# AILab-UniFI/GNN-TableExtraction

Measured on AMD Instinct MI355X. Metric: nodes/sec (fwd+bwd node classification) on PubLayNet page graphs, higher is better.
Workload: dtype f32 (GEMM operands split exactly into 3 bf16 pieces, fp32 accumulate)

## Files before the change

### gnn-tableextraction_amd/_lib.py

```python
from __future__ import annotations

import ctypes
import os
from ctypes import POINTER, c_char_p, c_float, c_int, c_int64, c_uint64, c_void_p

_HERE = os.path.dirname(os.path.abspath(__file__))
LIB_PATH = os.environ.get("GTE_LIB_PATH") or os.path.join(_HERE, "libgte_hip.so")

SIGNATURES = {
    "gte_version": (c_int, []),
    "gte_last_error": (c_char_p, []),
    "gte_device_info": (c_int, [c_void_p, c_void_p, c_void_p, c_void_p, c_int]),
    "gte_spmm_csr": (c_int, [c_void_p, c_void_p, c_void_p, c_void_p, c_int64, c_void_p, c_int64,
                             c_int64, c_int64, c_int, c_int, c_void_p]),
    "gte_spmm_csr_accumulate": (c_int, [c_void_p, c_void_p, c_void_p, c_void_p, c_int64, c_void_p, c_int64,
                                        c_int64, c_int64, c_int, c_int, c_void_p]),
    "gte_spmm_csr_edge_workspace_bytes": (c_int64, [c_int64, c_int64]),
    "gte_spmm_csr_edge": (c_int, [c_void_p, c_void_p, c_void_p, c_void_p, c_int64, c_void_p, c_int64, c_int64, c_int64, c_int64, c_int,
                                  c_void_p, c_int64, c_void_p]),
    "gte_spmm_tile_rows": (c_int, []),
    "gte_spmm_csr_tiled": (c_int, [c_void_p, c_void_p, c_void_p, c_void_p, c_void_p, c_void_p, c_void_p, c_int64,
                                   c_void_p, c_int64, c_int64, c_int64, c_int, c_int, c_void_p]),
    "gte_coo_to_csr_workspace_bytes": (c_int64, [c_int64, c_int64]),
    "gte_coo_to_csr": (c_int, [c_void_p, c_void_p, c_void_p, c_void_p, c_int64, c_int64,
# ... 68 lines not shown
                                        c_void_p, c_int64, c_int64, c_void_p]),
    "gte_sage_narrow_bwd_ln_p3_pad": (c_int, [c_void_p, c_int64, c_void_p, c_int64, c_void_p, c_int64, c_int64, c_int64, c_void_p, c_int64,
                                              c_int64, c_void_p, c_int64, c_void_p, c_int64, c_void_p, c_int64, c_void_p, c_int64, c_void_p,
                                              c_int64, c_void_p, c_float, c_void_p, c_void_p, c_int64, c_void_p, c_void_p, c_void_p, c_int,
                                              c_void_p, c_void_p, c_void_p, c_void_p, c_int64, c_void_p]),
    "gte_gemm_p3_nt_ln_bwd_supported": (c_int, [c_int64]),
    "gte_gemm_p3_nt_ln_bwd_workspace_bytes": (c_int64, [c_int64, c_int64]),
    "gte_gemm_p3_nt_ln_bwd": (c_int, [c_void_p, c_int64, c_int64, c_void_p, c_int64, c_int64, c_void_p, c_int64, c_void_p, c_int64,
                                      c_void_p, c_void_p, c_void_p, c_int, c_void_p, c_int64, c_void_p, c_int64, c_void_p, c_void_p,
                                      c_void_p, c_int64, c_int64, c_void_p, c_int64, c_void_p]),
    "gte_gemm_p3_nt_smallk_bwd_supported": (c_int, [c_int64, c_int64]),
    "gte_gemm_p3_nt_smallk_bwd_workspace_bytes": (c_int64, [c_int64, c_int64, c_int64]),
    "gte_gemm_p3_nt_smallk_bwd": (c_int, [c_void_p, c_int64, c_int64, c_void_p, c_int64, c_int64, c_void_p, c_int64, c_void_p, c_int64,
                                          c_int64, c_void_p, c_int64, c_int64, c_void_p, c_int64, c_void_p, c_void_p, c_void_p, c_void_p,
                                          c_int, c_void_p, c_int64, c_void_p, c_void_p, c_void_p, c_int64, c_int64, c_void_p, c_int64,
                                          c_void_p]),
    "gte_gemm_p3_nt_rows": (c_int, [c_void_p, c_int64, c_int64, c_void_p, c_int64, c_void_p, c_int64, c_void_p, c_int64,
                                    c_void_p, c_int64, c_int64, c_int64, c_int, c_int, c_void_p]),
    "gte_gemm_p3_tn_rows": (c_int, [c_void_p, c_int64, c_void_p, c_int64, c_void_p, c_int64, c_void_p, c_int64, c_int64, c_void_p,
                                    c_int64, c_int64, c_int64, c_int64, c_void_p, c_int64, c_void_p]),
    "gte_gemm_p3_nt_rows2": (c_int, [c_void_p, c_int64, c_void_p, c_int64, c_int64, c_void_p, c_int64, c_void_p, c_int64, c_void_p,
                                     c_int64, c_void_p, c_int64, c_int64, c_int64, c_int, c_int, c_void_p]),
    "gte_gemm_p3_tn_rows2": (c_int, [c_void_p, c_int64, c_void_p, c_int64, c_void_p, c_int64, c_void_p, c_int64, c_int64, c_void_p,
                                     c_int64, c_int64, c_int64, c_int64, c_void_p, c_int64, c_void_p]),
    "gte_gemm_p3_nt_ln_fwd_supported": (c_int, [c_int64]),
    "gte_gemm_p3_nt_ln_fwd": (c_int, [c_void_p, c_int64, c_int64, c_void_p, c_int64, c_int64, c_void_p, c_int64, c_void_p, c_void_p,
                                      c_void_p, c_float, c_int, c_void_p, c_int64, c_void_p, c_int64, c_void_p, c_int64, c_void_p,
                                      c_int64, c_int64, c_void_p]),
    "gte_gemm_p3_nt_rows2_ln_fwd": (c_int, [c_void_p, c_int64, c_void_p, c_int64, c_int64, c_void_p, c_int64, c_void_p, c_int64, c_void_p,
                                            c_void_p, c_void_p, c_float, c_int, c_void_p, c_int64, c_void_p, c_int64, c_void_p, c_int64,
                                            c_void_p, c_int64, c_int64, c_void_p]),
    "gte_gemm_p3_set_rows64": (c_int, [c_int]),
    "gte_gemm_p3_nt_plan": (c_int, [c_int64, c_int64, c_int64, c_int64, c_int, c_int, c_int, ctypes.POINTER(c_int)]),
    "gte_gemm_p3_set_nt_cfg": (c_int, [c_int]),
    "gte_gemm_p3_set_ln_rows": (c_int, [c_int]),
    "gte_batch_assemble_defer": (c_int, [c_int]),
    "gte_head_dlq_finish_workspace_bytes": (c_int64, [c_int64]),
    "gte_head_dlq_finish": (c_int, [c_void_p, c_void_p, c_void_p, c_void_p, c_int64, c_int64, c_int64, c_void_p, c_float, c_void_p,
                                    c_void_p, c_int64, c_void_p, c_void_p, c_int64, c_void_p]),
    "gte_gemm_p3_tn_workspace_bytes": (c_int64, [c_int64, c_int64, c_int64, c_int64]),
    "gte_gemm_p3_tn": (c_int, [c_void_p, c_int64, c_void_p, c_int64, c_void_p, c_int64, c_void_p, c_int64, c_int64, c_void_p,
                               c_int64, c_int64, c_int64, c_int64, c_void_p, c_int64, c_void_p]),
    "gte_adam_ticket_bytes": (c_int64, []),
    "gte_gcnsage_step": (c_int, [c_void_p, c_int, POINTER(c_int), c_void_p]),
    "gte_gcnsage_step_wide_layers": (c_int, [c_void_p]),
    "gte_gcnsage_forward": (c_int, [c_void_p, c_void_p]),
    "gte_fold_defer_begin": (c_int, [c_void_p]),
    "gte_fold_defer_flush": (c_int, []),
    "gte_fold_defer_flush_adam": (c_int, [c_void_p, c_void_p, c_void_p, c_void_p, c_int64, c_void_p, c_void_p, c_void_p, POINTER(c_int)]),
    "gte_fold_defer_flush_adam_images": (c_int, [c_void_p, c_void_p, c_void_p, c_void_p, c_int64, c_void_p, c_void_p, c_void_p, c_void_p,
                                                 c_int, POINTER(c_int)]),
    "gte_sage_transform_fwd": (c_int, [c_void_p, c_int64, c_int64, c_void_p, c_int64, c_void_p, c_int64, c_void_p, c_int64,
                                       c_int64, c_void_p]),
    "gte_sage_qform_dw_workspace_bytes": (c_int64, [c_int64, c_int64, c_int64]),
    "gte_sage_qform_dw": (c_int, [c_void_p, c_int64, c_void_p, c_int64, c_void_p, c_int64, c_int64, c_void_p, c_int64,
                                  c_int64, c_int64, c_void_p, c_int64, c_void_p]),
    "gte_sage_qform_dx": (c_int, [c_void_p, c_int64, c_void_p, c_int64, c_void_p, c_int64, c_int64, c_int64, c_void_p,
                                  c_int64, c_int64, c_void_p]),
    "gte_sage_narrow_supported": (c_int, [c_int64, c_int64]),
    "gte_sage_narrow_fwd": (c_int, [c_void_p, c_int64, c_int64, c_void_p, c_int64, c_void_p, c_int64, c_void_p, c_int64,
                                    c_void_p, c_int64, c_int64, c_void_p]),
    "gte_sage_narrow_fwd_ln_supported": (c_int, [c_int64, c_int64]),
    "gte_sage_narrow_fwd_ln": (c_int, [c_void_p, c_int64, c_int64, c_void_p, c_void_p, c_float, c_int, c_void_p, c_int64, c_void_p,
                                       c_void_p, c_int64, c_void_p, c_int64, c_void_p, c_int64, c_void_p, c_int64, c_int64,
                                       c_void_p]),
    "gte_sage_narrow_bwd_workspace_bytes": (c_int64, [c_int64, c_int64, c_int64]),
# ... 157 lines not shown
```

### gnn-tableextraction_amd/csrc/gemm_p3.hip

```cpp
#include "gte_common.h"
#include "gemm_p3_host.h"
#include "p3.h"
#include "smallk_step.h"

#include <stdlib.h>
#include <type_traits>
#include <utility>

namespace {

typedef __bf16 bf16x8 __attribute__((ext_vector_type(8)));
typedef float f32x16 __attribute__((ext_vector_type(16)));
typedef short s16x4 __attribute__((ext_vector_type(4)));
typedef __attribute__((address_space(3))) void* lds_ptr_t;
constexpr unsigned SRD_FLAGS = 0x00020000u;

template <typename F, int... I>
__device__ __forceinline__ void static_for_impl(F&& f, std::integer_sequence<int, I...>) {
    (f(std::integral_constant<int, I>{}), ...);
}
template <int N, typename F>
__device__ __forceinline__ void static_for(F&& f) {
    static_for_impl(static_cast<F&&>(f), std::make_integer_sequence<int, N>{});
}
// ... 532 lines not shown
                const long long rg = row_base + rlk;
                if (lane < kk && rlk < SR && rg < M) { p.lnf_stats[rg] = st_mean; p.lnf_stats[M + rg] = st_rstd; }
            }
        }
    } else {
        asm volatile("s_barrier" ::: "memory");
        static_assert(BN == 256, "whole rows per workgroup");
        constexpr int SR = TM * 32, LDT = 256;
        float* tile = reinterpret_cast<float*>(lds);
        constexpr bool MSK = LNB == 3;
        const int n = p.N, M = p.M;
        const int j4 = 4 * lane;
        const bool okc = MSK ? j4 < ((n + 3) & ~3) : j4 < n;
        bool oke[4];
        float gam[4], bet[4], s_dg[4], s_db[4], s_dbias[4];
#pragma unroll
        for (int e = 0; e < 4; ++e) {
            oke[e] = MSK ? j4 + e < n : okc;
            gam[e] = oke[e] ? p.ln_gamma[j4 + e] : 1.f;
            bet[e] = oke[e] ? p.ln_beta[j4 + e] : 0.f;
            s_dg[e] = s_db[e] = s_dbias[e] = 0.f;
        }
        const float inv_n = 1.0f / (float)n;
        const int col_l = lane & 31, hrow = (lane >> 5) * 4;
        constexpr int RF = 4;
        constexpr bool PRE = WM == 1;
        constexpr int RPW = PRE ? SR / NW : 1;
        constexpr int PD = RPW <= 12 ? RPW : 8;
        float zpre[PD][4], mpre[PD], rpre[PD];
        auto request_row = [&](int slot, int k) {
            const int rg = m0 + wave + k * NW;
            const int rc = rg < M ? rg : min(m0, M - 1);
            f4u zt; zt.x = zt.y = zt.z = zt.w = 0.f;
            if (okc) zt = *reinterpret_cast<const f4u*>(p.ln_z + (long long)rc * p.ln_ldz + j4);
            zpre[slot][0] = zt.x; zpre[slot][1] = zt.y; zpre[slot][2] = zt.z; zpre[slot][3] = zt.w;
            mpre[slot] = p.ln_stats[rc]; rpre[slot] = p.ln_stats[M + rc];
        };
        if constexpr (PRE) {
#pragma unroll
            for (int k = 0; k < PD; ++k) request_row(k, k);
        }
        for (int sl = 0; sl < WM; ++sl) {
            asm volatile("s_barrier" ::: "memory");
            if (wm == sl) {
#pragma unroll
                for (int b = 0; b < TN; ++b)
#pragma unroll
                    for (int a = 0; a < TM; ++a)
#pragma unroll
                        for (int r = 0; r < 16; ++r)
                            tile[(a * 32 + hrow + (r & 3) + 8 * (r >> 2)) * LDT + wn * (TN * 32) + b * 32 + col_l] = acc[a][b][r];
            }
            asm volatile("s_waitcnt lgkmcnt(0)\n\ts_barrier" ::: "memory");
            const int row_base = m0 + sl * SR;
            constexpr int ROUNDS = (SR + RF * NW - 1) / (RF * NW);
#pragma unroll
            for (int rd = 0; rd < ROUNDS; ++rd) {
                const int rl = wave + rd * RF * NW;
                if (rl >= SR) break;
                float gy[RF][4], zz[RF][4], mean[RF], rstd[RF];
                bool rok[RF];
#pragma unroll
                for (int u = 0; u < RF; ++u) {
                    const int rloc = rl + u * NW, rg = row_base + rloc;
                    rok[u] = rloc < SR && rg < M;
                    const int rc = rok[u] ? rg : min(row_base, M - 1);
                    float4 a = make_float4(0.f, 0.f, 0.f, 0.f), bz = a;
                    if (okc) {
                        if (rok[u]) a = *reinterpret_cast<const float4*>(tile + rloc * LDT + j4);
// ... 4 lines not shown
                    }
                    gy[u][0] = a.x; gy[u][1] = a.y; gy[u][2] = a.z; gy[u][3] = a.w;
                    if constexpr (PRE) {
                        const int k = rd * RF + u;
                        const int e_ = (k < RPW ? k : 0) % PD;
#pragma unroll
                        for (int e = 0; e < 4; ++e) zz[u][e] = zpre[e_][e];
                        mean[u] = mpre[e_]; rstd[u] = rpre[e_];
                        if (k + PD < RPW) request_row(e_, k + PD);
                    } else {
                        zz[u][0] = bz.x; zz[u][1] = bz.y; zz[u][2] = bz.z; zz[u][3] = bz.w;
                        mean[u] = p.ln_stats[rc]; rstd[u] = p.ln_stats[M + rc];
                    }
                }
                float dd[RF][4];
#pragma unroll
                for (int u = 0; u < RF; ++u) {
#pragma unroll
                    for (int e = 0; e < 4; ++e) dd[u][e] = 0.f;
                    if (!rok[u]) continue;
                    const long long rg = row_base + rl + u * NW;
                    float xh[4], g[4];
                    float a = 0.f, b = 0.f;
                    if constexpr (MSK) gte_ln_bwd_pre4m(gy[u], zz[u], mean[u], rstd[u], gam, bet, oke, p.ln_relu, xh, g, a, b);
                    else gte_ln_bwd_pre4(gy[u], zz[u], mean[u], rstd[u], gam, bet, okc, p.ln_relu, xh, g, a, b);
                    const float c1 = gte_group_sum<64>(a) * inv_n, c2 = gte_group_sum<64>(b) * inv_n;
                    if constexpr (MSK) gte_ln_bwd_post4m(g, xh, gam, rstd[u], c1, c2, oke, dd[u], s_dg, s_db, s_dbias);
                    else gte_ln_bwd_post4(g, xh, gam, rstd[u], c1, c2, okc, dd[u], s_dg, s_db, s_dbias);
                    if (okc && p.ln_dz) {
                        f4u o; o.x = dd[u][0]; o.y = dd[u][1]; o.z = dd[u][2]; o.w = dd[u][3];
                        *reinterpret_cast<f4u*>(p.ln_dz + rg * p.ln_lddz + j4) = o;
                    }
                }
                if (p.ln_dzp3) {
                    const bool odd = lane & 1;
                    const int col0 = 4 * (lane & ~1);
                    const bool im8 = MSK ? col0 < ((n + 15) & ~15) : col0 < n;
#pragma unroll
                    for (int u = 0; u < RF; u += 2) {
                        float x[8];
#pragma unroll
                        for (int e = 0; e < 4; ++e) {
                            const float got = gte_quad_swap1(odd ? dd[u][e] : dd[u + 1][e]);
                            x[e] = odd ? got : dd[u][e];
                            x[4 + e] = odd ? dd[u + 1][e] : got;
                        }
                        if (im8 && rok[odd ? u + 1 : u])
                            p3::store8(p.ln_dzp3 + (long long)(row_base + rl + (odd ? u + 1 : u) * NW) * p.ln_ldp3, col0, x);
                    }
                }
            }
        }
        asm volatile("s_waitcnt lgkmcnt(0)\n\ts_barrier" ::: "memory");
        float* red = reinterpret_cast<float*>(lds);
#pragma unroll
        for (int e = 0; e < 4; ++e) {
            red[(wave * 3 + 0) * 256 + j4 + e] = s_dg[e];
            red[(wave * 3 + 1) * 256 + j4 + e] = s_db[e];
            red[(wave * 3 + 2) * 256 + j4 + e] = s_dbias[e];
        }
        asm volatile("s_waitcnt lgkmcnt(0)\n\ts_barrier" ::: "memory");
        float* pp = p.ln_part + (long long)lb * 3 * n;
        for (int i = tid; i < 3 * 256; i += NW * 64) {
            const int q = i >> 8, j = i & 255;
            float v = 0.f;
#pragma unroll
            for (int w = 0; w < NW; ++w) v += red[(w * 3 + q) * 256 + j];
            if (j < n) pp[q * n + j] = v;
        }
    }
}

template <int WM, int WN, int TM, int TN, int NL, int LNB = 0, bool BIG = false>
__global__ void __launch_bounds__((WM * WN + NL) * 64, (WM * WN + NL + 3) / 4)
gemm_p3_nt_lw_kernel(const P3Gemm p) {
    constexpr int NW = WM * WN, NBUF = 3;
    constexpr int BM = WM * TM * 32, BN = WN * TN * 32;
    constexpr int A_INST = BM * 96 / 1024, B_INST = BN * 96 / 1024, N_INST = A_INST + B_INST;
    constexpr int A_BYTES = BM * 96;
    constexpr int NI = (N_INST + NL - 1) / NL;
    constexpr int STAGE = NI * NL * 1024;
    extern __shared__ __attribute__((aligned(16))) char lds[];

// ... 121 lines not shown
#if P3_ABL & 16
    const long long c0 = __builtin_amdgcn_s_memtime(), r0 = __builtin_amdgcn_s_memrealtime();
#endif
#if P3_ABL & 4
    F f;
    read_frags(f, lds);
#endif
    for (int t = 0; t < T; ++t) {
#if !(P3_ABL & 4)
        F f;
        read_frags(f, lds + rd * STAGE);
#endif
#if P3_ABL & 8
        keep_frags<TM, TN>(f);
#else
        products<TM, TN>(acc, f);
#endif
        asm volatile("s_waitcnt lgkmcnt(0)\n\ts_barrier" ::: "memory");
        rd = rd + 1 == NBUF ? 0 : rd + 1;
    }
#if P3_ABL & 16
    if (tid == 0 && p.slab) {
        long long* st = reinterpret_cast<long long*>(p.slab) + 2 * blockIdx.x;
        st[0] = __builtin_amdgcn_s_memtime() - c0;
        st[1] = __builtin_amdgcn_s_memrealtime() - r0;
    }
#endif
#if P3_ABL & 32
    if (p.K != 12345) return;
#endif
    lw_epilogue<WM, WN, TM, TN, LNB>(acc, lds, p, m0, n0, lb, wave, lane, tid);
}

template <int TM, int NL, int LNB = 0, int SQ = 4>
__global__ void __launch_bounds__((8 + NL) * 64, (8 + NL + 3) / 4)
gemm_p3_nt_sq_kernel(const P3Gemm p) {
    constexpr int WM = 1, WN = 8, TN = 1, NW = 8, NSLOT = 3;
    constexpr int BM = TM * 32, BN = 256;
    constexpr int G = BM * 96 / 1024;
    constexpr int NG = (G + NL - 1) / NL;
    constexpr int NIQ = NG * SQ;
    constexpr int BLK = BM * 96, SLOT = SQ * BLK;
    static_assert(SQ == 4 && BLK % 1024 == 0 && NIQ <= 24, "slot");
    extern __shared__ __attribute__((aligned(16))) char lds[];

    const int tid = threadIdx.x, lane = tid & 63;
    const int wave = __builtin_amdgcn_readfirstlane(tid >> 6);
    const int tiles_n = (p.N + BN - 1) / BN;
    const unsigned lb = gte_xcd_remap(blockIdx.x, gridDim.x);
    const int tm = (int)(lb / (unsigned)tiles_n), tn = (int)(lb % (unsigned)tiles_n);
    const int m0 = tm * BM, n0 = tn * BN;
    const int KB1 = p.KB1, T = p.KB1 + p.KB2;
    const int S = (T + SQ - 1) / SQ;

    if (wave >= NW) {
        const int lw = wave - NW;
        const int rowsA = min(BM, p.M - m0);
        const int lda1 = (int)p.lda1, lda2 = (int)(p.A2 ? p.lda2 : p.lda1);
        const char* baseA1 = p.rowsA ? p.A1 : p.A1 + (long long)m0 * p.lda1;
        const char* baseA2 = p.A2 ? (p.rows_both ? p.A2 : p.A2 + (long long)m0 * p.lda2) : baseA1;
        const int recA1 = p.rowsA ? (int)(unsigned)p.res_bytes : rowsA * lda1;
        const int recA2 = p.rows_both ? (int)(unsigned)p.res_bytes2 : rowsA * lda2;
        constexpr int OOB = (int)0xfffffc00u;
        char* const scratch = lds + NSLOT * SLOT;
        int vo1[NG], vo2[NG];
        static_for<NG>([&](auto GI) {
            constexpr int g = decltype(GI)::value;
            const int gi = g * NL + lw;
            const int sl = gi * 64 + lane, row = sl / 6, part = sl - row * 6, sp = part ^ ((row >> 3) & 1);
            vo1[g] = gi >= G ? OOB : row * lda1 + sp * 16;
            vo2[g] = gi >= G ? OOB : row * lda2 + sp * 16;
            if (p.rowsA && gi < G) {
                const int rr = row < rowsA ? p.rowsA[m0 + row] : -1;
                vo1[g] = rr < 0 ? OOB : (int)((unsigned)rr * (unsigned)lda1 + (unsigned)(sp * 16));
                if (p.rows_both) vo2[g] = rr < 0 ? OOB : (int)((unsigned)rr * (unsigned)lda2 + (unsigned)(sp * 16));
            }
        });
        const __amdgpu_buffer_rsrc_t sa1 = __builtin_amdgcn_make_buffer_rsrc(const_cast<char*>(baseA1), 0, recA1, SRD_FLAGS);
        const __amdgpu_buffer_rsrc_t sa2 = __builtin_amdgcn_make_buffer_rsrc(const_cast<char*>(baseA2), 0, recA2, SRD_FLAGS);
        auto issue = [&](int s, char* slot) {
            static_for<NG>([&](auto GI) {
                constexpr int g = decltype(GI)::value;
                const int gi = g * NL + lw;
                static_for<SQ>([&](auto QI) {
                    constexpr int q = decltype(QI)::value;
#if P3_ABL & 1
                    if (s >= 2) return;
#endif
                    const int t = s * SQ + q;
                    const bool seg = t >= KB1;
                    const int vo = seg ? vo2[g] : vo1[g];
                    dma16(seg ? sa2 : sa1, gi < G ? slot + q * BLK + gi * 1024 : scratch,
                          (t < T && vo != OOB) ? vo + (seg ? t - KB1 : t) * 96 : OOB);
                });
            });
        };
        issue(0, lds);
        issue(1, lds + SLOT);
        wait_dma_barrier<NIQ>();
        int wr = 2;
        for (int s = 0; s < S; ++s) {
            issue(s + 2, lds + wr * SLOT);
            wr = wr + 1 == NSLOT ? 0 : wr + 1;
            wait_dma_barrier<NIQ>();
        }
        if constexpr (LNB != 0) asm volatile("s_waitcnt vmcnt(0)\n\ts_barrier" ::: "memory");
        return;
    }
    const int wn = wave;
    const int r = lane & 31, hsel = lane >> 5;
    const int a_rd = r * 96 + (hsel ^ ((r >> 3) & 1)) * 16;
    const int rowsB = min(BN, p.N - n0);
    const char* const baseB = p.B + (long long)n0 * 96;
    const int b_vo = (wn * 32 + r) * 96 + hsel * 16;
    const long long bsb = p.bsb;
    bf16x8 bq[4][3];
    auto load_b = [&](bf16x8 (&dst)[3], int t, bool valid) {
        const __amdgpu_buffer_rsrc_t sb = __builtin_amdgcn_make_buffer_rsrc(const_cast<char*>(baseB + (long long)min(t, T - 1) * bsb), 0,
                                                                            valid ? rowsB * 96 : 0, SRD_FLAGS);
        static_for<3>([&](auto PL) {
            constexpr int pl = decltype(PL)::value;
            dst[pl] = __builtin_bit_cast(bf16x8, __builtin_amdgcn_raw_buffer_load_b128(sb, b_vo + pl * 32, 0, 0));
        });
    };
    f32x16 acc[TM][1];
#pragma unroll
    for (int a = 0; a < TM; ++a)
#pragma unroll
        for (int e = 0; e < 16; ++e) acc[a][0][e] = 0.f;
    auto block = [&](const char* blk, const bf16x8 (&b)[3]) {
        bf16x8 fa[3][TM];
        static_for<3>([&](auto GQ) {
            constexpr int g = decltype(GQ)::value;
// ... 26 lines not shown
    auto nvalid = [&](int s) { return s >= S ? 0 : min(SQ, T - s * SQ); };
    int k0 = 0, nv = nvalid(0);
    load_b(bq[0], 0, 0 < nv);
    load_b(bq[1], 1, 1 < nv);
    load_b(bq[2], 2, 2 < nv);
    asm volatile("s_barrier" ::: "memory");
#if P3_ABL & 16
    const long long c0 = __builtin_amdgcn_s_memtime(), r0 = __builtin_amdgcn_s_memrealtime();
#endif
    int rd = 0;
    for (int s = 0; s < S; ++s) {
        const char* slot = lds + rd * SLOT;
        const int k1 = kfirst(s + 1), nv1 = nvalid(s + 1);
        static_for<SQ>([&](auto J) {
            constexpr int j = decltype(J)::value;
            if constexpr (j + 3 < SQ) load_b(bq[(j + 3) & 3], k0 + j + 3, j + 3 < nv);
            else load_b(bq[(j + 3) & 3], k1 + j + 3 - SQ, j + 3 - SQ < nv1);
            block(slot + j * BLK, bq[j]);
        });
        asm volatile("s_waitcnt lgkmcnt(0)\n\ts_barrier" ::: "memory");
        rd = rd + 1 == NSLOT ? 0 : rd + 1;
        k0 = k1; nv = nv1;
    }
#if P3_ABL & 16
    if (tid == 0 && p.slab) {
        long long* st = reinterpret_cast<long long*>(p.slab) + 2 * blockIdx.x;
        st[0] = __builtin_amdgcn_s_memtime() - c0;
        st[1] = __builtin_amdgcn_s_memrealtime() - r0;
    }
#endif
#if P3_ABL & 32
    if (p.K != 12345) return;
#endif
    lw_epilogue<WM, WN, TM, TN, LNB>(acc, lds, p, m0, n0, lb, wave, lane, tid);
}

#ifndef P3_TN_ABL
#define P3_TN_ABL 0
#endif
template <int WM, int WN, int WGS, bool MAP = false, bool BIG = false>
__global__ void __launch_bounds__(WM * WN * 64, (WM * WN * WGS + 3) / 4)
gemm_p3_tn_kernel(const P3Gemm p) {
    static_assert(!BIG || MAP, "64-bit rows: the row-mapped kernel");
    static_assert(!MAP || (WM == 2 && WN == 2), "row map: the 128 x 128 tile");
    constexpr int NW = WM * WN, TM = 2, TN = 2;
    constexpr int BM = WM * 64, BN = WN * 64, NBA = BM / 16, NBB = BN / 16;
    constexpr int RSA = NBA * 96, RSB = NBB * 96;
    constexpr int A_BYTES = 16 * RSA, B_BYTES = 16 * RSB;
    constexpr int A_INST = A_BYTES / 1024, B_INST = B_BYTES / 1024, N_INST = A_INST + B_INST;
    constexpr int NI = (N_INST + NW - 1) / NW;
    constexpr int STAGE = NI * NW * 1024;
    static_assert((NBA & (NBA - 1)) == 0 && (NBB & (NBB - 1)) == 0 && NBA >= 8 && NBB >= 8, "blocks per row: a power of two >= 8");
    extern __shared__ __attribute__((aligned(16))) char lds[];

    const int tid = threadIdx.x, lane = tid & 63;
    const int wave = __builtin_amdgcn_readfirstlane(tid >> 6);
    const int wm = wave / WN, wn = wave % WN;

    const int nsegs = p.Nseg > 0 ? 2 : 1, seg_cols = p.Nseg > 0 ? p.Nseg : p.N;
    const int seg_tiles = (seg_cols + BN - 1) / BN, tiles_n = nsegs * seg_tiles, tiles_m = (p.M + BM - 1) / BM;
    const unsigned ntile = (unsigned)(tiles_m * tiles_n);
    const unsigned lu = gte_xcd_remap(blockIdx.x, gridDim.x);
    const int split = (int)(lu / ntile);
    const unsigned lb = lu % ntile;
    const int tm = (int)(lb / (unsigned)tiles_n), tn = (int)(lb % (unsigned)tiles_n);
    const int nseg = tn / seg_tiles;
    const int m0 = tm * BM, n0 = (tn % seg_tiles) * BN;
// ... 379 lines not shown
    p.bsa1 = p.bsa2 = 96; p.bsb = sb.bs;
    p.M = (int)m; p.N = (int)n; p.splits = 1;
    if (o.rows) {
        p.rowsA = o.rows; p.res_bytes = o.n_res_rows * o.lda1;
        if (o.k2 > 0) { p.rows_both = 1; p.res_bytes2 = o.n_res_rows * o.lda2; }
        p.rows64 = (rows64_needed(p.res_bytes) || (o.k2 > 0 && rows64_needed(p.res_bytes2))) ? 1 : 0;
    }
    return GTE_OK;
}

template <int WM, int WN, int TM, int TN, int NBUF, int WGS>
void launch_ring(const P3Gemm& p, hipStream_t s) {
    constexpr int NW = WM * WN, BM = WM * TM * 32, BN = WN * TN * 32;
    constexpr int NI = ((BM + BN) * 96 / 1024 + NW - 1) / NW, shm = NBUF * NI * NW * 1024;
    static bool configured = false;
    set_lds_once(configured, &gemm_p3_nt_ring_kernel<WM, WN, TM, TN, NBUF, WGS>, shm);
    const dim3 grid((unsigned)(gte::ceil_div(p.M, BM) * gte::ceil_div(p.N, BN)));
    hipLaunchKernelGGL((gemm_p3_nt_ring_kernel<WM, WN, TM, TN, NBUF, WGS>), grid, dim3(NW * 64), shm, s, p);
}
template <int WM, int WN, int TM, int TN, int NL, int LNB = 0, bool BIG = false>
void launch_lw(const P3Gemm& p, hipStream_t s) {
    constexpr int BM = WM * TM * 32, BN = WN * TN * 32;
    constexpr int NI = ((BM + BN) * 96 / 1024 + NL - 1) / NL, shm = 3 * NI * NL * 1024;
    static_assert(LNB == 0 || (BN == 256 && shm >= TM * 32 * 256 * 4 && shm >= WM * WN * 3 * 256 * 4),
                  "the epilogue's row slice lives in the stage images");
    static bool configured = false;
    set_lds_once(configured, &gemm_p3_nt_lw_kernel<WM, WN, TM, TN, NL, LNB, BIG>, shm);
    const dim3 grid((unsigned)(gte::ceil_div(p.M, BM) * gte::ceil_div(p.N, BN)));
    hipLaunchKernelGGL((gemm_p3_nt_lw_kernel<WM, WN, TM, TN, NL, LNB, BIG>), grid, dim3((WM * WN + NL) * 64), shm, s, p);
}
template <int TM, int NL, int LNB>
void launch_sq(const P3Gemm& p, hipStream_t s) {
    constexpr int BM = TM * 32, shm = 3 * 4 * BM * 96 + 1024;
    static_assert(LNB == 0 || (shm >= BM * 256 * 4 && shm >= 8 * 3 * 256 * 4), "the epilogue's row slice lives in the slots");
    static bool configured = false;
    set_lds_once(configured, &gemm_p3_nt_sq_kernel<TM, NL, LNB>, shm);
    const dim3 grid((unsigned)(gte::ceil_div(p.M, BM) * gte::ceil_div(p.N, 256)));
    hipLaunchKernelGGL((gemm_p3_nt_sq_kernel<TM, NL, LNB>), grid, dim3((8 + NL) * 64), shm, s, p);
}

inline bool sq_applies(const P3Gemm& p) {
    if (p.ldb != 96 || p.bsb < 96 || p.rows64 || p.N > 256 || p.bsa1 != 96 || p.bsa2 != 96) return false;
    const int T = p.KB1 + p.KB2, S4 = 4 * ((T + 3) / 4);
    return T >= 32 && (S4 - T) * 12 <= T;
}
inline bool sq_plain_wanted(const P3Gemm& p) { return p.N > 128; }
struct NtCfg { int id, bm, bn, wgs; };
constexpr NtCfg kNtCfg[] = {{0, 64, 128, 3}, {1, 128, 128, 2}, {2, 128, 256, 1}, {3, 160, 256, 1}, {4, 192, 256, 1}, {5, 224, 256, 1},
                            {6, 256, 256, 1}};
thread_local int g_nt_cfg = -2;
int nt_choose(const P3Gemm& p, int cus) {
    const int forced = g_nt_cfg;
    if (forced >= 0 && forced <= 7) return forced;
    double best = 1e30;
    int bi = 0;
    for (const NtCfg& c : kNtCfg) {
        if (p.N <= 128 && c.bn > 128) continue;
        const int64_t tiles = gte::ceil_div(p.M, c.bm) * gte::ceil_div(p.N, c.bn);
        const int64_t rounds = gte::ceil_div(tiles, (int64_t)cus * c.wgs);
        const double penalty = c.bm * c.bn >= 128 * 256 ? 1.0 : (c.bm * c.bn >= 128 * 128 ? 1.15 : 1.35);
        const double t = (double)rounds * c.wgs * c.bm * c.bn * penalty;
        if (t < best) { best = t; bi = c.id; }
    }
    return bi;
}
inline int one_round_row_tile(int64_t m, int64_t cus, int min_tile = 32) {
    for (int t = 32; t <= 96; t += 32)
// ... 108 lines not shown
                              int relu, int accumulate, void* stream) {
    return gte::gemm_p3_nt({a1, lda1, k1, a2, lda2, k2, b, ldb, nullptr, 0}, bias, bias_cols, c, ldc, m, n, relu, accumulate, stream);
}

extern "C" int gte_gemm_p3_nt_rows(const void* a_res, int64_t ldpa, int64_t k, const int32_t* a_rows, int64_t n_res_rows, const void* b,
                                   int64_t ldpb, const float* bias, int64_t bias_cols, float* c, int64_t ldc, int64_t m, int64_t n,
                                   int relu, int accumulate, void* stream) {
    if (!a_rows) return gte::fail(GTE_ERR_INVALID_ARGUMENT, "gemm_p3_nt_rows: null row map");
    return gte::gemm_p3_nt({a_res, ldpa, k, nullptr, 0, 0, b, ldpb, a_rows, n_res_rows}, bias, bias_cols, c, ldc, m, n, relu, accumulate,
                           stream, "gemm_p3_nt_rows");
}

extern "C" int gte_gemm_p3_nt_rows2(const void* a_res, int64_t ldpa, const void* a2_res, int64_t ldpa2, int64_t k, const int32_t* a_rows,
                                    int64_t n_res_rows, const void* b, int64_t ldpb, const float* bias, int64_t bias_cols, float* c,
                                    int64_t ldc, int64_t m, int64_t n, int relu, int accumulate, void* stream) {
    if (!a_rows || !a2_res) return gte::fail(GTE_ERR_INVALID_ARGUMENT, "gemm_p3_nt_rows2: null row map / second image");
    return gte::gemm_p3_nt({a_res, ldpa, k, a2_res, ldpa2, k, b, ldpb, a_rows, n_res_rows}, bias, bias_cols, c, ldc, m, n, relu, accumulate,
                           stream, "gemm_p3_nt_rows2");
}

extern "C" int gte_gemm_p3_nt_plan(int64_t m, int64_t n, int64_t k1, int64_t k2, int weights_block_major, int epilogue, int cus,
                                   int* row_tile) {
    if (row_tile) *row_tile = 0;
    if (m <= 0 || n <= 0 || k1 <= 0 || k2 < 0 || (epilogue != 0 && epilogue != 1 && epilogue != 3 && epilogue != 4))
        return gte::fail(GTE_ERR_INVALID_ARGUMENT, "gemm_p3_nt_plan: bad arguments (epilogue: 0 plain, 1 / 3 LayerNorm backward, 4 LayerNorm forward)");
    P3Gemm p = {};
    p.M = (int)m; p.N = (int)n; p.KB1 = (int)p3::blocks(k1); p.KB2 = (int)p3::blocks(k2);
    p.bsa1 = p.bsa2 = 96;
    p.ldb = weights_block_major ? 96 : (p.KB1 + p.KB2) * 96; p.bsb = weights_block_major ? gte::round_up(n, 16) * 96 : 96;
    const NtPick k = nt_pick(p, epilogue, cus);
    const bool sq = k.family == NtFamily::sq;
    if (row_tile && n <= 256 && (epilogue != 0 || sq)) *row_tile = k.bm;
    return sq ? 1 : 0;
}

extern "C" int gte_gemm_p3_set_nt_cfg(int cfg) {
    if (cfg < -1 || cfg > 7) return gte::fail(GTE_ERR_INVALID_ARGUMENT, "gemm_p3_set_nt_cfg: -1 (chooser) or a configuration id 0 ... 7");
    g_nt_cfg = cfg;
    return GTE_OK;
}

extern "C" int gte_gemm_p3_set_ln_rows(int rows) {
    if (rows != 0 && rows != 32 && rows != 64 && rows != 96 && rows != 128)
        return gte::fail(GTE_ERR_INVALID_ARGUMENT, "gemm_p3_set_ln_rows: 0 (chooser), 32, 64, 96 or 128");
    g_ln_rows = rows;
    return GTE_OK;
}
extern "C" int gte_gemm_p3_nt_ln_bwd_supported(int64_t n) { return (n >= 1 && n <= 256) ? 1 : 0; }
extern "C" int64_t gte_gemm_p3_nt_ln_bwd_workspace_bytes(int64_t m, int64_t n) {
    if (m <= 0 || n <= 0) return 256;
    return gte::round_up(gte::ceil_div(m, 32) * 3 * n * 4, 256);
}
int gte::gemm_p3_nt_ln_bwd(const P3NtOperands& op, const float* z, int64_t ldz, const float* stats, const float* gamma, const float* beta,
                           int relu, float* dz, int64_t lddz, void* dzp3, int64_t ldp3, float* dgamma, float* dbeta, float* dbias,
                           int64_t m, int64_t n, void* workspace, int64_t workspace_bytes, void* stream) {
    const char* name = "gemm_p3_nt_ln_bwd";
    const int64_t n4 = gte::round_up(n, 4);
    NtLimits lim = {};
    lim.max_ld = 1 << 23; lim.below_2gb = true;
    lim.own_sizes = n <= 0 || op.k1 > INT32_MAX || op.k2 > INT32_MAX;
    lim.unsupported = gte_gemm_p3_nt_ln_bwd_supported(n) ? nullptr : "needs n <= 256";
    lim.own_null = !z || !stats || !gamma || !beta || (!dz && !dzp3) || !workspace;
    lim.own_ld = ldz < n4 || (dz && lddz < n4) || (dzp3 && (ldp3 < p3::row_bytes(n) || ldp3 % 16 != 0));
    P3Gemm p = {};
    int rc = nt_prepare(name, op, m, n, lim, p);
    if (rc != GTE_OK || p.M == 0) return rc;
// ... 210 lines not shown
```

### include/gte.h

```cpp
#ifndef GTE_H_
#define GTE_H_

#include <stdint.h>

#ifdef __cplusplus
extern "C" {
#endif

#define GTE_VERSION 400

enum gte_status {
    GTE_OK = 0,
    GTE_ERR_INVALID_ARGUMENT = -1,
    GTE_ERR_LAUNCH = -2,
    GTE_ERR_WORKSPACE_TOO_SMALL = -3,
    GTE_ERR_UNSUPPORTED = -4,
};

enum gte_reduce { GTE_REDUCE_SUM = 0, GTE_REDUCE_MEAN = 1 };
enum gte_dtype { GTE_F32 = 0, GTE_BF16 = 1 };

int gte_version(void);
const char* gte_last_error(void);
int gte_device_info(int* compute_units, int* wave_size, int* lds_bytes, char* arch_name, int arch_name_len);
// ... 151 lines not shown
int gte_gemm_p3_nt_rows2_ln_fwd(const void* a_res, int64_t ldpa, const void* a2_res, int64_t ldpa2, int64_t k, const int32_t* a_rows,
                                int64_t n_res_rows, const void* b, int64_t ldpb, const float* bias, const float* gamma,
                                const float* beta, float eps, int relu, float* z, int64_t ldz, float* y, int64_t ldy, void* yp3,
                                int64_t ldyp3, float* stats, int64_t m, int64_t n, void* stream);
int gte_gemm_p3_nt_ln_bwd_supported(int64_t n);
int64_t gte_gemm_p3_nt_ln_bwd_workspace_bytes(int64_t m, int64_t n);
int gte_gemm_p3_nt_ln_bwd(const void* a1, int64_t ldpa1, int64_t k1, const void* a2, int64_t ldpa2, int64_t k2, const void* b,
                          int64_t ldpb, const float* z, int64_t ldz, const float* stats, const float* gamma, const float* beta,
                          int relu, float* dz, int64_t lddz, void* dzp3, int64_t ldp3, float* dgamma, float* dbeta, float* dbias,
                          int64_t m, int64_t n, void* workspace, int64_t workspace_bytes, void* stream);
int gte_gemm_p3_nt_smallk_bwd_supported(int64_t k_total, int64_t n);
int64_t gte_gemm_p3_nt_smallk_bwd_workspace_bytes(int64_t m, int64_t k_total, int64_t n);
int gte_gemm_p3_nt_smallk_bwd(const void* a1, int64_t ldpa1, int64_t kg1, const void* a2, int64_t ldpa2, int64_t kg2, const void* b,
                              int64_t ldpb, const float* x, int64_t ldx, int64_t k1, const float* ahn, int64_t ldahn, int64_t k2,
                              const float* W, int64_t ldw, const float* bias, const float* gamma, const float* beta,
                              const float* stats, int relu, float* dW, int64_t lddw, float* dbias, float* dgamma, float* dbeta,
                              int64_t m, int64_t n, void* workspace, int64_t workspace_bytes, void* stream);
int64_t gte_gemm_p3_tn_workspace_bytes(int64_t m, int64_t n, int64_t nseg, int64_t k);
int gte_gemm_p3_tn(const void* a, int64_t ldpa, const void* a2, int64_t ldpa2, const void* b, int64_t ldpb, const void* b2,
                   int64_t ldpb2, int64_t nseg, float* c, int64_t ldc, int64_t m, int64_t n, int64_t k, void* workspace,
                   int64_t workspace_bytes, void* stream);

int gte_gemm_p3_tn_rows(const void* a, int64_t ldpa, const void* a2, int64_t ldpa2, const void* b_res, int64_t ldpb,
                        const int32_t* b_rows, int64_t n_res_rows, int64_t nseg, float* c, int64_t ldc, int64_t m, int64_t n,
                        int64_t k, void* workspace, int64_t workspace_bytes, void* stream);
int gte_gemm_p3_tn_rows2(const void* a, int64_t ldpa, const void* b_res, int64_t ldpb, const void* b2_res, int64_t ldpb2,
                         const int32_t* b_rows, int64_t n_res_rows, int64_t nseg, float* c, int64_t ldc, int64_t m, int64_t n,
                         int64_t k, void* workspace, int64_t workspace_bytes, void* stream);
int64_t gte_head_dlq_finish_workspace_bytes(int64_t n_nodes);
int gte_head_dlq_finish(const int32_t* rindptr, const int32_t* rindices, const float* w_out, const float* dlq, int64_t lddlq,
                        int64_t n_nodes, int64_t n_classes, const void* ce_partial, float grad_scale, float* out3, void* dlqp3,
                        int64_t ldp, float* gbias, void* workspace, int64_t workspace_bytes, void* stream);
int gte_gemm_p3_nt_plan(int64_t m, int64_t n, int64_t k1, int64_t k2, int weights_block_major, int epilogue, int cus, int* row_tile);
int gte_gemm_p3_set_nt_cfg(int cfg);
int gte_gemm_p3_set_ln_rows(int rows);
int gte_gemm_p3_set_rows64(int mode);
int gte_batch_assemble_rows(const int32_t* pages, int64_t n_batch, const int32_t* node_off, const int32_t* b_node_off,
                            const gte_batch_arrays* in_edges, const gte_batch_arrays* out_edges, const float* feat,
                            int64_t ld_feat, int64_t n_cols, float* feat_out, const float* label, float* label_out,
                            int64_t n_out, int32_t* row_map, int64_t row_map_pad, int64_t n_res_rows, void* stream);

int gte_dropout_mask(float p, uint64_t seed, int rank, int64_t step, int site, int64_t n_rows, int64_t n_cols, uint8_t* mask,
                     int64_t ldm, void* stream);
int gte_dropout_mask_host(float p, uint64_t seed, int rank, int64_t step, int site, int64_t n_rows, int64_t n_cols, uint8_t* mask,
                          int64_t ldm);
#define GTE_DROPOUT_MAX_ROWS ((int64_t)1 << 30)
int gte_dropout_set_wide(int mode);
int gte_dropout_get_wide(void);
int gte_spmm_dropout_p3(const int32_t* indptr, const int32_t* indices, const float* eweight, const float* x, int64_t ldx,
                        const void* xp, int64_t ldpx, const int32_t* x_rows, int64_t n_res_rows, int in_dropout, float p, uint64_t seed,
                        int rank, const int64_t* step_counter, int site, void* selfp3, int64_t ldp_self, void* aggp3, int64_t ldp_agg,
                        int64_t n_rows, int64_t n_feat, void* stream);
int gte_spmm_dropout_bwd(const int32_t* rindptr, const int32_t* rindices, const float* w_out, const float* g, int64_t ldg,
                         int64_t agg_col, float p, uint64_t seed, int rank, const int64_t* step_counter, int site, float* dx,
                         int64_t lddx, int64_t n_rows, int64_t n_feat, void* stream);

enum gte_layer_kind { GTE_LAYER_PLANES = 0, GTE_LAYER_SMALLK = 1, GTE_LAYER_AGGFIRST = 2, GTE_LAYER_CACHED = 3, GTE_LAYER_DROPOUT = 4 };
typedef struct gte_step_layer {
    int kind;
    int64_t fin, fout;
    const float* W; const float* bias; const float* gamma; const float* beta; float eps; int relu;
    float* gW; float* gbias; float* ggamma; float* gbeta;
    void* wimg_fwd; int64_t ldp_wfwd;
    void* wimg_bwd; int64_t ldp_wbwd;
    const float* x; int64_t ldx;
    void* hp; int64_t ldp_h;
// ... 190 lines not shown
```

Baseline: 49.36 million.

## Split LayerNorm-backward epilogue across all twelve waves including loader waves

The LN-backward epilogue of the square NT GEMM kernel is now shared by all twelve waves: the four loader waves, which previously sat idle after their last DMA, take a row share alongside the eight compute waves. Each wave prefetches its rows' z values and statistics before the final barrier, and the accumulator tile is staged to LDS before the rows are processed. This aims to shorten the serial epilogue tail and hide the z/stat loads behind the GEMM. In exchange it adds register pressure for the prefetched rows and extra barriers, plus ablation macros, a row-share query API and profiling tools.

```diff
diff --git a/gnn-tableextraction_amd/_lib.py b/gnn-tableextraction_amd/_lib.py
--- a/gnn-tableextraction_amd/_lib.py
+++ b/gnn-tableextraction_amd/_lib.py
@@ -124,6 +124,7 @@
                                             c_void_p, c_int64, c_int64, c_void_p]),
     "gte_gemm_p3_set_rows64": (c_int, [c_int]),
     "gte_gemm_p3_nt_plan": (c_int, [c_int64, c_int64, c_int64, c_int64, c_int, c_int, c_int, ctypes.POINTER(c_int)]),
+    "gte_gemm_p3_ln_bwd_row_share": (c_int, [c_int, c_int, ctypes.POINTER(c_int), ctypes.POINTER(c_int)]),
     "gte_gemm_p3_set_nt_cfg": (c_int, [c_int]),
     "gte_gemm_p3_set_ln_rows": (c_int, [c_int]),
     "gte_batch_assemble_defer": (c_int, [c_int]),
diff --git a/gnn-tableextraction_amd/csrc/gemm_p3.hip b/gnn-tableextraction_amd/csrc/gemm_p3.hip
--- a/gnn-tableextraction_amd/csrc/gemm_p3.hip
+++ b/gnn-tableextraction_amd/csrc/gemm_p3.hip
@@ -588,9 +588,13 @@
             const int rg = m0 + wave + k * NW;
             const int rc = rg < M ? rg : min(m0, M - 1);
             f4u zt; zt.x = zt.y = zt.z = zt.w = 0.f;
+#if P3_ABL & 256
+            zt.x = (float)(rc + lane); mpre[slot] = 0.f; rpre[slot] = 1.f;
+#else
             if (okc) zt = *reinterpret_cast<const f4u*>(p.ln_z + (long long)rc * p.ln_ldz + j4);
+            mpre[slot] = p.ln_stats[rc]; rpre[slot] = p.ln_stats[M + rc];
+#endif
             zpre[slot][0] = zt.x; zpre[slot][1] = zt.y; zpre[slot][2] = zt.z; zpre[slot][3] = zt.w;
-            mpre[slot] = p.ln_stats[rc]; rpre[slot] = p.ln_stats[M + rc];
         };
         if constexpr (PRE) {
 #pragma unroll
@@ -661,6 +665,7 @@
                         *reinterpret_cast<f4u*>(p.ln_dz + rg * p.ln_lddz + j4) = o;
                     }
                 }
+#if !(P3_ABL & 512)
                 if (p.ln_dzp3) {
                     const bool odd = lane & 1;
                     const int col0 = 4 * (lane & ~1);
@@ -678,6 +683,7 @@
                             p3::store8(p.ln_dzp3 + (long long)(row_base + rl + (odd ? u + 1 : u) * NW) * p.ln_ldp3, col0, x);
                     }
                 }
+#endif
             }
         }
         asm volatile("s_waitcnt lgkmcnt(0)\n\ts_barrier" ::: "memory");
@@ -865,6 +871,132 @@
     lw_epilogue<WM, WN, TM, TN, LNB>(acc, lds, p, m0, n0, lb, wave, lane, tid);
 }
 
+constexpr int LNB12_CW = 8, LNB12_LW = 4, LNB12_WAVES = LNB12_CW + LNB12_LW;
+struct LnbShare { int first, rows; };
+constexpr __host__ __device__ LnbShare lnb_row_share(int tile_rows, int wave) {
+    const int c = 2 * (tile_rows / (2 * LNB12_WAVES)), l = (tile_rows - LNB12_CW * c) / LNB12_LW;
+    return wave < LNB12_CW ? LnbShare{wave * c, c} : LnbShare{LNB12_CW * c + (wave - LNB12_CW) * l, l};
+}
+template <int R>
+struct LnbRows { float z[R][4]; float mean, rstd; };
+template <int R, bool MSK>
+__device__ __forceinline__ void lnb12_request(LnbRows<R>& q, const P3Gemm& p, int row0, int lane) {
+    static_assert(R >= 1 && R <= 64, "a row's statistics per lane");
+    const int n = p.N, M = p.M, j4 = 4 * lane;
+    const bool okc = MSK ? j4 < ((n + 3) & ~3) : j4 < n;
+#if P3_ABL & 256
+#pragma unroll
+    for (int k = 0; k < R; ++k) q.z[k][0] = q.z[k][1] = q.z[k][2] = q.z[k][3] = (float)(row0 + k + lane);
+    q.mean = 0.f; q.rstd = 1.f;
+    (void)M; (void)okc;
+#else
+#pragma unroll
+    for (int k = 0; k < R; ++k) {
+        const int rc = min(row0 + k, M - 1);
+        f4u zt; zt.x = zt.y = zt.z = zt.w = 0.f;
+        if (okc) zt = *reinterpret_cast<const f4u*>(p.ln_z + (long long)rc * p.ln_ldz + j4);
+        q.z[k][0] = zt.x; q.z[k][1] = zt.y; q.z[k][2] = zt.z; q.z[k][3] = zt.w;
+    }
+    const int rs = min(row0 + min(lane, R - 1), M - 1);
+    q.mean = p.ln_stats[rs]; q.rstd = p.ln_stats[M + rs];
+#endif
+}
+template <int LNB, int R>
+__device__ __forceinline__ void lnb12_rows(const LnbRows<R>& q, char* lds, const P3Gemm& p, int m0, unsigned lb, int wave, int first,
+                                           int lane, int tid) {
+    constexpr bool MSK = LNB == 3;
+    constexpr int LDT = 256, RF = 4, NW = LNB12_WAVES;
+    const float* tile = reinterpret_cast<const float*>(lds);
+    const int n = p.N, M = p.M;
+    const int j4 = 4 * lane;
+    const bool okc = MSK ? j4 < ((n + 3) & ~3) : j4 < n;
+    bool oke[4];
+    float gam[4], bet[4], s_dg[4], s_db[4], s_dbias[4];
+#pragma unroll
+    for (int e = 0; e < 4; ++e) {
+        oke[e] = MSK ? j4 + e < n : okc;
+        gam[e] = oke[e] ? p.ln_gamma[j4 + e] : 1.f;
+        bet[e] = oke[e] ? p.ln_beta[j4 + e] : 0.f;
+        s_dg[e] = s_db[e] = s_dbias[e] = 0.f;
+    }
+    const float inv_n = 1.0f / (float)n;
+    const int row_base = m0 + first;
+    constexpr int ROUNDS = (R + RF - 1) / RF;
+#pragma unroll
+    for (int rd = 0; rd < ROUNDS; ++rd) {
+        float gy[RF][4], dd[RF][4];
+        bool rok[RF];
+#pragma unroll
+        for (int u = 0; u < RF; ++u) {
+            const int k = rd * RF + u;
+            rok[u] = k < R && row_base + k < M;
+            float4 a = make_float4(0.f, 0.f, 0.f, 0.f);
+            if (okc && rok[u]) a = *reinterpret_cast<const float4*>(tile + (first + k) * LDT + j4);
+            gy[u][0] = a.x; gy[u][1] = a.y; gy[u][2] = a.z; gy[u][3] = a.w;
+        }
+#pragma unroll
+        for (int u = 0; u < RF; ++u) {
+#pragma unroll
+            for (int e = 0; e < 4; ++e) dd[u][e] = 0.f;
+            const int k = rd * RF + u < R ? rd * RF + u : 0;
+            if (!rok[u]) continue;
+            const long long rg = row_base + k;
+            const float mean = __builtin_bit_cast(float, __builtin_amdgcn_readlane(__builtin_bit_cast(int, q.mean), k));
+            const float rstd = __builtin_bit_cast(float, __builtin_amdgcn_readlane(__builtin_bit_cast(int, q.rstd), k));
+            float xh[4], g[4];
+            float a = 0.f, b = 0.f;
+            if constexpr (MSK) gte_ln_bwd_pre4m(gy[u], q.z[k], mean, rstd, gam, bet, oke, p.ln_relu, xh, g, a, b);
+            else gte_ln_bwd_pre4(gy[u], q.z[k], mean, rstd, gam, bet, okc, p.ln_relu, xh, g, a, b);
+            const float c1 = gte_group_sum<64>(a) * inv_n, c2 = gte_group_sum<64>(b) * inv_n;
+            if constexpr (MSK) gte_ln_bwd_post4m(g, xh, gam, rstd, c1, c2, oke, dd[u], s_dg, s_db, s_dbias);
+            else gte_ln_bwd_post4(g, xh, gam, rstd, c1, c2, okc, dd[u], s_dg, s_db, s_dbias);
+            if (okc && p.ln_dz) {
+                f4u o; o.x = dd[u][0]; o.y = dd[u][1]; o.z = dd[u][2]; o.w = dd[u][3];
+                *reinterpret_cast<f4u*>(p.ln_dz + rg * p.ln_lddz + j4) = o;
+            }
+        }
+#if !(P3_ABL & 512)
+        if (p.ln_dzp3) {
+            const bool odd = lane & 1;
+            const int col0 = 4 * (lane & ~1);
+            const bool im8 = MSK ? col0 < ((n + 15) & ~15) : col0 < n;
+#pragma unroll
+            for (int u = 0; u < RF; u += 2) {
+                float x[8];
+#pragma unroll
+                for (int e = 0; e < 4; ++e) {
+                    const float got = gte_quad_swap1(odd ? dd[u][e] : dd[u + 1][e]);
+                    x[e] = odd ? got : dd[u][e];
+                    x[4 + e] = odd ? dd[u + 1][e] : got;
+                }
+                if (im8 && rok[odd ? u + 1 : u])
+                    p3::store8(p.ln_dzp3 + (long long)(row_base + rd * RF + (odd ? u + 1 : u)) * p.ln_ldp3, col0, x);
+            }
+        }
+#endif
+    }
+    asm volatile("s_waitcnt lgkmcnt(0)\n\ts_barrier" ::: "memory");
+    float* red = reinterpret_cast<float*>(lds);
+#pragma unroll
+    for (int e = 0; e < 4; ++e) {
+        red[(wave * 3 + 0) * 256 + j4 + e] = s_dg[e];
+        red[(wave * 3 + 1) * 256 + j4 + e] = s_db[e];
+        red[(wave * 3 + 2) * 256 + j4 + e] = s_dbias[e];
+    }
+    asm volatile("s_waitcnt lgkmcnt(0)\n\ts_barrier" ::: "memory");
+    float* pp = p.ln_part + (long long)lb * 3 * n;
+    static_assert(NW * 64 == 3 * 256, "one column sum per thread");
+    const int qd = tid >> 8, j = tid & 255;
+    float v = 0.f;
+#pragma unroll
+    for (int w = 0; w < NW; ++w) v += red[(w * 3 + qd) * 256 + j];
+    if (j < n) pp[qd * n + j] = v;
+}
+
+#ifndef P3_EPI8
+#define P3_EPI8 0
+#endif
+
 template <int TM, int NL, int LNB = 0, int SQ = 4>
 __global__ void __launch_bounds__((8 + NL) * 64, (8 + NL + 3) / 4)
 gemm_p3_nt_sq_kernel(const P3Gemm p) {
@@ -885,6 +1017,9 @@
     const int m0 = tm * BM, n0 = tn * BN;
     const int KB1 = p.KB1, T = p.KB1 + p.KB2;
     const int S = (T + SQ - 1) / SQ;
+    constexpr bool EPI12 = (LNB == 1 || LNB == 3) && NL == LNB12_LW && !P3_EPI8 && !(P3_ABL & 32);
+    constexpr int RC = lnb_row_share(BM, 0).rows, RL = lnb_row_share(BM, LNB12_CW).rows;
+    static_assert(!EPI12 || (RC >= 1 && RC <= 12 && RL >= 1 && LNB12_CW * RC + LNB12_LW * RL == BM), "the row shares cover the tile");
 
     if (wave >= NW) {
         const int lw = wave - NW;
@@ -932,6 +1067,22 @@
         issue(1, lds + SLOT);
         wait_dma_barrier<NIQ>();
         int wr = 2;
+        if constexpr (EPI12) {
+            for (int s = 0; s < S - 1; ++s) {
+                issue(s + 2, lds + wr * SLOT);
+                wr = wr + 1 == NSLOT ? 0 : wr + 1;
+                wait_dma_barrier<NIQ>();
+            }
+            issue(S + 1, lds + wr * SLOT);
+            const LnbShare sh = lnb_row_share(BM, wave);
+            LnbRows<RL> q;
+            lnb12_request<RL, LNB == 3>(q, p, m0 + sh.first, lane);
+            wait_dma_barrier<NIQ>();
+            asm volatile("s_waitcnt vmcnt(0)\n\ts_barrier" ::: "memory");
+            asm volatile("s_barrier" ::: "memory");
+            lnb12_rows<LNB, RL>(q, lds, p, m0, lb, wave, sh.first, lane, tid);
+            return;
+        }
         for (int s = 0; s < S; ++s) {
             issue(s + 2, lds + wr * SLOT);
             wr = wr + 1 == NSLOT ? 0 : wr + 1;
@@ -1024,7 +1175,22 @@
 #if P3_ABL & 32
     if (p.K != 12345) return;
 #endif
-    lw_epilogue<WM, WN, TM, TN, LNB>(acc, lds, p, m0, n0, lb, wave, lane, tid);
+    if constexpr (EPI12) {
+        const LnbShare sh = lnb_row_share(BM, wave);
+        LnbRows<RC> q;
+        lnb12_request<RC, LNB == 3>(q, p, m0 + sh.first, lane);
+        asm volatile("s_barrier" ::: "memory");
+        float* tile = reinterpret_cast<float*>(lds);
+        const int col_l = lane & 31, hrow = (lane >> 5) * 4;
+#pragma unroll
+        for (int a = 0; a < TM; ++a)
+#pragma unroll
+            for (int r = 0; r < 16; ++r) tile[(a * 32 + hrow + (r & 3) + 8 * (r >> 2)) * 256 + wn * 32 + col_l] = acc[a][0][r];
+        asm volatile("s_waitcnt lgkmcnt(0)\n\ts_barrier" ::: "memory");
+        lnb12_rows<LNB, RC>(q, lds, p, m0, lb, wave, sh.first, lane, tid);
+    } else {
+        lw_epilogue<WM, WN, TM, TN, LNB>(acc, lds, p, m0, n0, lb, wave, lane, tid);
+    }
 }
 
 #ifndef P3_TN_ABL
@@ -1470,7 +1636,7 @@
 template <int TM, int NL, int LNB>
 void launch_sq(const P3Gemm& p, hipStream_t s) {
     constexpr int BM = TM * 32, shm = 3 * 4 * BM * 96 + 1024;
-    static_assert(LNB == 0 || (shm >= BM * 256 * 4 && shm >= 8 * 3 * 256 * 4), "the epilogue's row slice lives in the slots");
+    static_assert(LNB == 0 || (shm >= BM * 256 * 4 && shm >= LNB12_WAVES * 3 * 256 * 4), "the epilogue's row slice lives in the slots");
     static bool configured = false;
     set_lds_once(configured, &gemm_p3_nt_sq_kernel<TM, NL, LNB>, shm);
     const dim3 grid((unsigned)(gte::ceil_div(p.M, BM) * gte::ceil_div(p.N, 256)));
@@ -1645,6 +1811,14 @@
     const bool sq = k.family == NtFamily::sq;
     if (row_tile && n <= 256 && (epilogue != 0 || sq)) *row_tile = k.bm;
     return sq ? 1 : 0;
+}
+
+extern "C" int gte_gemm_p3_ln_bwd_row_share(int tile_rows, int wave, int* first_row, int* rows) {
+    if ((tile_rows != 32 && tile_rows != 64 && tile_rows != 96 && tile_rows != 128) || wave < 0 || wave >= LNB12_WAVES || !first_row || !rows)
+        return gte::fail(GTE_ERR_INVALID_ARGUMENT, "gemm_p3_ln_bwd_row_share: tile rows 32 / 64 / 96 / 128, wave 0 ... 11");
+    const LnbShare sh = lnb_row_share(tile_rows, wave);
+    *first_row = sh.first; *rows = sh.rows;
+    return GTE_OK;
 }
 
 extern "C" int gte_gemm_p3_set_nt_cfg(int cfg) {
diff --git a/include/gte.h b/include/gte.h
--- a/include/gte.h
+++ b/include/gte.h
@@ -207,6 +207,7 @@
                         int64_t n_nodes, int64_t n_classes, const void* ce_partial, float grad_scale, float* out3, void* dlqp3,
                         int64_t ldp, float* gbias, void* workspace, int64_t workspace_bytes, void* stream);
 int gte_gemm_p3_nt_plan(int64_t m, int64_t n, int64_t k1, int64_t k2, int weights_block_major, int epilogue, int cus, int* row_tile);
+int gte_gemm_p3_ln_bwd_row_share(int tile_rows, int wave, int* first_row, int* rows);
 int gte_gemm_p3_set_nt_cfg(int cfg);
 int gte_gemm_p3_set_ln_rows(int rows);
 int gte_gemm_p3_set_rows64(int mode);
diff --git a/profiles/debug/kernel_medians.py b/profiles/debug/kernel_medians.py
--- /dev/null
+++ b/profiles/debug/kernel_medians.py
@@ -0,0 +1,24 @@
+import re
+import sqlite3
+import statistics
+import sys
+
+args = sys.argv[1:]
+min_calls = 20
+if args and args[0] == "--min-calls":
+    min_calls, args = int(args[1]), args[2:]
+tags, table = [], {}
+for a in args:
+    tag, path = a.split("=", 1)
+    tags.append(tag)
+    per = {}
+    for name, dur in sqlite3.connect(path).execute("select name, end - start from kernels"):
+        name = re.sub(r"\s+", " ", re.sub(r"\(anonymous namespace\)::", "", name))
+        name = re.sub(r"^void ", "", name.split("(")[0])[:70]
+        per.setdefault(name, []).append(dur / 1e3)
+    for name, d in per.items():
+        if len(d) >= min_calls:
+            table.setdefault(name, {})[tag] = (statistics.median(d), len(d))
+print(f"{'kernel (median us; calls)':72s}" + "".join(f"{t:>18s}" for t in tags))
+for name in sorted(table, key=lambda k: -max(v[0] * v[1] for v in table[k].values())):
+    print(f"{name:72s}" + "".join(f"{table[name][t][0]:11.2f} ({table[name][t][1]:4d})" if t in table[name] else f"{'-':>18s}" for t in tags))
diff --git a/profiles/micro/dx_ln_abl.hip b/profiles/micro/dx_ln_abl.hip
--- /dev/null
+++ b/profiles/micro/dx_ln_abl.hip
@@ -0,0 +1,85 @@
+#include "../../gnn-tableextraction_amd/csrc/gemm_p3.hip"
+
+#include <algorithm>
+#include <cstdio>
+#include <cstring>
+#include <vector>
+
+bool gte::wide_forced() { return false; }
+
+__global__ void fill_kernel(float* x, long long n, unsigned seed, float scale, float shift) {
+    long long i = (long long)blockIdx.x * 256 + threadIdx.x;
+    if (i >= n) return;
+    unsigned h = (unsigned)i * 2654435761u + seed;
+    h ^= h >> 16; h *= 0x7feb352du; h ^= h >> 15; h *= 0x846ca68bu; h ^= h >> 16;
+    x[i] = ((int)(h & 0xffffff) - 0x800000) * (1.0f / 0x800000) * scale + shift;
+}
+static void fill(float* x, long long n, unsigned seed, float scale = 1.f, float shift = 0.f) {
+    fill_kernel<<<(unsigned)((n + 255) / 256), 256>>>(x, n, seed, scale, shift);
+}
+
+int main(int argc, char** argv) {
+    const long long M = argc > 1 ? atoll(argv[1]) : 24437, N = 256, K = 256;
+    const int rows = getenv("ABL_ROWS") ? atoi(getenv("ABL_ROWS")) : 96;
+    const long long lda = gte_p3_row_bytes(K), ldw = 256 * 96, ldo = gte_p3_row_bytes(N);
+    float *tmp, *z, *stats, *gamma, *beta, *part;
+    char *a1, *a2, *w, *dzp;
+    long long* stamps;
+    hipMalloc(&tmp, M * 2 * K * 4); hipMalloc(&z, M * 2 * N * 4); hipMalloc(&stats, 2 * M * 4);
+    hipMalloc(&gamma, 1024); hipMalloc(&beta, 1024); hipMalloc(&part, gte_gemm_p3_nt_ln_bwd_workspace_bytes(M, N));
+    hipMalloc(&a1, M * lda); hipMalloc(&a2, M * lda); hipMalloc(&w, 2 * (K / 16) * ldw); hipMalloc(&dzp, M * ldo);
+    hipMalloc(&stamps, 4096 * 16);
+    hipMemset(stamps, 0, 4096 * 16);
+    fill(tmp, M * K, 1u); gte_p3_from_f32(tmp, K, M, K, 0, a1, lda, nullptr);
+    fill(tmp, M * K, 7u); gte_p3_from_f32(tmp, K, M, K, 0, a2, lda, nullptr);
+    fill(tmp, N * 2 * K, 3u, 1.f / 16);
+    for (int fb = 0; fb < 2 * K / 16; ++fb) gte_p3_from_f32(tmp + 16 * fb, 2 * K, N, 16, 0, w + fb * ldw, 96, nullptr);
+    fill(z, M * 2 * N, 5u); fill(stats, M, 9u, 0.1f); fill(stats + M, M, 10u, 0.2f, 1.f);
+    fill(gamma, 256, 12u, 0.1f, 1.f); fill(beta, 256, 13u, 0.1f);
+    hipDeviceSynchronize();
+
+    P3Gemm p = {};
+    p.A1 = a1; p.lda1 = lda; p.KB1 = (int)(K / 16); p.A2 = a2; p.lda2 = lda; p.KB2 = p.KB1;
+    p.B = w; p.ldb = 96; p.bsb = ldw; p.bsa1 = p.bsa2 = 96;
+    p.M = (int)M; p.N = (int)N; p.splits = 1;
+    p.ln_z = z; p.ln_ldz = 2 * N; p.ln_stats = stats; p.ln_gamma = gamma; p.ln_beta = beta; p.ln_relu = 1;
+    p.ln_dz = nullptr; p.ln_dzp3 = dzp; p.ln_ldp3 = ldo; p.ln_part = part;
+    p.slab = reinterpret_cast<float*>(stamps);
+    auto launch = [&] {
+        if (rows == 96) launch_sq<3, 4, 1>(p, nullptr); else launch_sq<4, 4, 1>(p, nullptr);
+    };
+    std::vector<double> us;
+    for (int rep = 0; rep < 5; ++rep) {
+        hipEvent_t e0, e1;
+        hipEventCreate(&e0); hipEventCreate(&e1);
+        for (int i = 0; i < (rep ? 100 : 2000); ++i) launch();
+        hipEventRecord(e0);
+        for (int i = 0; i < 300; ++i) launch();
+        hipEventRecord(e1);
+        if (hipDeviceSynchronize() != hipSuccess) { printf("launch failed: %s\n", hipGetErrorString(hipGetLastError())); return 1; }
+        float ms = 0.f;
+        hipEventElapsedTime(&ms, e0, e1);
+        us.push_back(ms * 1e3 / 300);
+        hipEventDestroy(e0); hipEventDestroy(e1);
+    }
+    std::sort(us.begin(), us.end());
+    const double gf = 2.0 * M * N * 2 * K * 1e-9;
+    printf("dX + LN bwd %lld x %lld x %lld, %3d-row tiles, %s epilogue, abl %3d: %6.1f us (min %.1f max %.1f of 5 x 300)  %.3f of 416.7 TF",
+           M, N, 2 * K, rows == 96 ? 96 : 128, P3_EPI8 ? "eight-wave " : "twelve-wave", P3_ABL, us[2], us.front(), us.back(), gf / us[2] * 1e3 / 416.7);
+#if P3_ABL & 16
+    {
+        const int bm = rows == 96 ? 96 : 128, nwg = (int)((M + bm - 1) / bm);
+        std::vector<long long> h(4096 * 2);
+        hipMemcpy(h.data(), stamps, 4096 * 16, hipMemcpyDeviceToHost);
+        std::vector<double> ghz, t;
+        for (int i = 0; i < nwg; ++i)
+            if (h[2 * i + 1] > 0) { ghz.push_back((double)h[2 * i] / (double)h[2 * i + 1] * 0.1); t.push_back((double)h[2 * i + 1] * 0.01); }
+        if (!t.empty()) {
+            std::sort(ghz.begin(), ghz.end()); std::sort(t.begin(), t.end());
+            printf("  in-kernel: clock %.3f GHz, K loop median %.1f us (min %.1f max %.1f)", ghz[ghz.size() / 2], t[t.size() / 2], t.front(), t.back());
+        }
+    }
+#endif
+    printf("\n");
+    return 0;
+}
```

After: 49.48 million (median of 6 runs). No clear change (+0.2%).
